# qiskit-community/adapt-aqc

Hardware: AMD Instinct MI355X
Metric: overlap+gradient evals/sec, 50-qubit MPS chi=64, 1/2/4/8 MI355X (higher is better)
Workload: dtype c128

## Files before the change

### adaptaqc_amd/csrc/svd_gram.h

```cpp
#pragma once

constexpr int kGramMaxK = 128;
constexpr int kGramNarrowK = 64;
constexpr double kGramRelFloor = 1e-9;
__device__ unsigned long long g_gram_ticks[12];
static_assert(kGramNarrowK == 64, "S5: the narrow inverse iteration (tid < K) stays on wave 0");
__device__ unsigned long long g_gram_stats[6];

__device__ __forceinline__ double wave_sum_d(double v) {
#pragma unroll
  for (int off = 32; off > 0; off >>= 1) v += __shfl_xor(v, off);
  return v;
}

__device__ __forceinline__ double wave_sum_dpp(double v) {
  v = aqc::row_sum16(v);
  double s = 0.0;
#pragma unroll
  for (int rr = 0; rr < 4; ++rr) {
    const int lo = __builtin_amdgcn_readlane(__double2loint(v), 16 * rr);
    const int hi = __builtin_amdgcn_readlane(__double2hiint(v), 16 * rr);
    s += __hiloint2double(hi, lo);
  }
  return s;
}

__device__ __forceinline__ cplx pick16(const cplx (&g)[16], int i) {
  switch (i) {
#define AQC_PICK(n) \
  case n:           \
    return g[n];
    AQC_PICK(0) AQC_PICK(1) AQC_PICK(2) AQC_PICK(3) AQC_PICK(4) AQC_PICK(5) AQC_PICK(6) AQC_PICK(7)
    AQC_PICK(8) AQC_PICK(9) AQC_PICK(10) AQC_PICK(11) AQC_PICK(12) AQC_PICK(13) AQC_PICK(14)
#undef AQC_PICK
    default:
      return g[15];
  }
}

__device__ __forceinline__ double uniform_d(double v) {
  const int lo = __builtin_amdgcn_readfirstlane(__double2loint(v));
  const int hi = __builtin_amdgcn_readfirstlane(__double2hiint(v));
  return __hiloint2double(hi, lo);
}

__device__ __forceinline__ double bcast_d(double v, int l) {
  const int lo = __builtin_amdgcn_readlane(__double2loint(v), l);
  const int hi = __builtin_amdgcn_readlane(__double2hiint(v), l);
  return __hiloint2double(hi, lo);
}

__device__ __forceinline__ int fresh_lane() {
  int l = __builtin_amdgcn_mbcnt_hi(~0u, __builtin_amdgcn_mbcnt_lo(~0u, 0u));
  asm volatile("" : "+v"(l));
  return l;
}
template <class T>
__device__ __forceinline__ T* uniform_ptr(T* p) {
  const unsigned long long a = (unsigned long long)p;
  const unsigned lo = __builtin_amdgcn_readfirstlane((unsigned)a);
  const unsigned hi = __builtin_amdgcn_readfirstlane((unsigned)(a >> 32));
  return (T*)(((unsigned long long)hi << 32) | lo);
}
__device__ __forceinline__ int sign_bit(double q) { return (int)((unsigned)__double2hiint(q) >> 31); }

__device__ __forceinline__ int sturm_count_poly(const double2* de, int C, double xn) {
  double p0 = 1.0, p1 = de[0].x - xn;
  int s1 = __double2hiint(p1) >> 31;
  int neg = s1;
  int i = 1;
  auto step = [&](double2 e) {
    const double p2 = fma(e.x - xn, p1, -(e.y * p0));
    const int s2 = __double2hiint(p2) >> 31;
    neg += s1 ^ s2;
    s1 = s2;
    p0 = p1;
    p1 = p2;
  };
  auto rescale = [&]() {
    const int ex = max(__builtin_amdgcn_frexp_exp(p0), __builtin_amdgcn_frexp_exp(p1));
    p0 = __builtin_amdgcn_ldexp(p0, -ex);
    p1 = __builtin_amdgcn_ldexp(p1, -ex);
  };
  auto rd4 = [&](int i0, double2& r0, double2& r1, double2& r2, double2& r3) {
    r0 = de[min(i0, C - 1)], r1 = de[min(i0 + 1, C - 1)], r2 = de[min(i0 + 2, C - 1)], r3 = de[min(i0 + 3, C - 1)];
  };
  double2 a0, a1, a2, a3, b0, b1, b2, b3;
  rd4(1, a0, a1, a2, a3);
  for (; i + 8 <= C; i += 8) {
    rd4(i + 4, b0, b1, b2, b3);
    __builtin_amdgcn_sched_barrier(0);
    step(a0);
    step(a1);
    step(a2);
    step(a3);
    rescale();
    rd4(i + 8, a0, a1, a2, a3);
    __builtin_amdgcn_sched_barrier(0);
    step(b0);
    step(b1);
    step(b2);
    step(b3);
    rescale();
  }
  if (i + 4 <= C) {
    step(a0);
    step(a1);
    step(a2);
    step(a3);
    rescale();
    i += 4;
  }
  for (; i < C; ++i) step(de[i]);
  return -neg;
}

__device__ __forceinline__ double rcp_nr(double x) {
  double r = __builtin_amdgcn_rcp(x);
  r = r * fma(-x, r, 2.0);
  r = r * fma(-x, r, 2.0);
  return r;
}

constexpr size_t kTfacOff = 16384;
constexpr size_t kWideOff = 20480;
static_assert(kWideOff + 8192 <= aqc::kGramWorkElems, "Gram-path scratch exceeds the work buffer");
static_assert(kChainLdsBytes >= 128 * 128 * 8, "S5 (K > 64): 128 x 128 vectors in the dynamic LDS");
typedef __attribute__((address_space(1))) double gdbl_t;

__device__ __forceinline__ void s6_factors(int b, int C, cplx* hh, const cplx* s_tau, int lane) {
  const int k1 = C - 1 - 16 * b, k0 = k1 > 16 ? k1 - 16 : 0, nb = k1 - k0;
  const int li = lane & 15, lk = lane >> 4;
  aqc::d4_t sr = {0, 0, 0, 0}, si = {0, 0, 0, 0};
  for (int r0 = 0; r0 < C; r0 += 4) {
    const int row = r0 + lk, k = k0 + li;
    const cplx y = (li < nb && row > k && row < C) ? aqc::ldg(hh + (size_t)k * (2 * C - k - 1) / 2 + (row - k - 1))
                                                   : aqc::cmk(0, 0);
    sr = __builtin_amdgcn_mfma_f64_16x16x4f64(y.x, y.x, sr, 0, 0, 0);
    sr = __builtin_amdgcn_mfma_f64_16x16x4f64(y.y, y.y, sr, 0, 0, 0);
    si = __builtin_amdgcn_mfma_f64_16x16x4f64(y.x, y.y, si, 0, 0, 0);
    si = __builtin_amdgcn_mfma_f64_16x16x4f64(-y.y, y.x, si, 0, 0, 0);
  }
  cplx* Sg = hh + kTfacOff + (size_t)b * 512;
#pragma unroll
  for (int q = 0; q < 4; ++q) aqc::stg(Sg + (lk + 4 * q) * 16 + li, aqc::cmk(sr[q], si[q]));
  asm volatile("s_waitcnt vmcnt(0)" ::: "memory");
  const int a = lane >> 2, g = lane & 3;
  cplx tq[4] = {aqc::cmk(0, 0), aqc::cmk(0, 0), aqc::cmk(0, 0), aqc::cmk(0, 0)};
  for (int i = 0; i < 16; ++i) {
    const cplx tau = i < nb ? s_tau[k0 + i] : aqc::cmk(0, 0);
    cplx acc = aqc::cmk(0, 0);
#pragma unroll
    for (int m = 0; m < 4; ++m) {
      const int bb = g + 4 * m;
      if (4 * m < i && bb < i) {
        const gdbl_t* sp = (const gdbl_t*)(const double*)(Sg + bb * 16 + i);
        const cplx sv = aqc::cmk(__hip_atomic_load(sp, __ATOMIC_RELAXED, __HIP_MEMORY_SCOPE_AGENT),
                                 __hip_atomic_load(sp + 1, __ATOMIC_RELAXED, __HIP_MEMORY_SCOPE_AGENT));
        acc = aqc::cfma(tq[m], sv, acc);
      }
    }
    acc.x = aqc::row_sum4(acc.x);
    acc.y = aqc::row_sum4(acc.y);
    const cplx ti = aqc::cmul(tau, acc);
    const cplx val = a < i ? aqc::cmk(-ti.x, -ti.y) : (a == i ? tau : aqc::cmk(0, 0));
    if (g == (i & 3)) tq[i >> 2] = val;
  }
#pragma unroll
  for (int m = 0; m < 4; ++m) aqc::stg(Sg + 256 + a * 16 + g + 4 * m, tq[m]);
}

template <int ZS>
__device__ __forceinline__ void gs_clusters(int K, int C, double* zb, const double* s_lam, double s_tn, int lane) {
  const double ortol = 1e-7 * s_tn;
  int start = 0;
  for (int i = 1; i < K; ++i) {
    if (s_lam[i - 1] - s_lam[i] >= ortol) {
      start = i;
      continue;
    }
    for (int jj = start; jj < i; ++jj) {
      double dp = 0.0;
      for (int row = lane; row < C; row += 64) dp = fma(zb[row * ZS + i], zb[row * ZS + jj], dp);
      dp = wave_sum_d(dp);
      for (int row = lane; row < C; row += 64) zb[row * ZS + i] = fma(-dp, zb[row * ZS + jj], zb[row * ZS + i]);
    }
    double n2 = 0.0;
    for (int row = lane; row < C; row += 64) n2 = fma(zb[row * ZS + i], zb[row * ZS + i], n2);
    n2 = wave_sum_d(n2);
    const double sc = 1.0 / sqrt(n2);
    for (int row = lane; row < C; row += 64) zb[row * ZS + i] *= sc;
  }
}

template <int ZS>
__device__ __forceinline__ double rayleigh(int i, int C, const double* zb, const double* s_d, const double* s_e) {
  double s2a = 0.0, s2b = 0.0;
  int r0 = 0;
  constexpr int U = 8;
  for (; r0 + U <= C; r0 += U) {
    double zz[U + 1], dd[U], ee[U];
#pragma unroll
    for (int u = 0; u <= U; ++u) zz[u] = zb[min(r0 + u, C - 1) * ZS + i];
#pragma unroll
    for (int u = 0; u < U; ++u) dd[u] = s_d[r0 + u], ee[u] = r0 + u < C - 1 ? s_e[r0 + u] : 0.0;
#pragma unroll
    for (int u = 0; u < U; ++u) {
      s2a = fma(dd[u] * zz[u], zz[u], s2a);
      s2b = fma(2.0 * ee[u] * zz[u], zz[u + 1], s2b);
    }
  }
  for (; r0 < C; ++r0) {
    const double z = zb[r0 * ZS + i];
    s2a = fma(s_d[r0] * z, z, s2a);
    if (r0 < C - 1) s2b = fma(2.0 * s_e[r0] * z, zb[(r0 + 1) * ZS + i], s2b);
  }
  const double s2 = s2a + s2b;
  return s2 > 0.0 ? s2 : 0.0;
}

__device__ __forceinline__ void s6_back(const TwoSiteJob& j, cplx* hh, int C, int K, int c0, aqc::d4_t (&vre)[2],
                                        aqc::d4_t (&vim)[2], const double* s_sig2, int tid, int lane, int wave,
                                        int wave_s) {
  extern __shared__ double2 xbuf[];
  const int nt = wave & 3, mg = wave >> 2, li = lane & 15, lk = lane >> 4;
  cplx* Yl = xbuf;
  cplx* Pw = Yl + 2048;
  cplx* Tl = Pw + 12 * 256;
  cplx* W2l = Tl + 3 * 256 + 16 * 64;
  auto fetch_y = [&](int k0, int nb, cplx (&y)[2]) {
#pragma unroll
    for (int u = 0; u < 2; ++u) {
      const int e = tid + 1024 * u, row = e >> 4, i = e & 15, k = k0 + i;
      y[u] = (i < nb && row > k && row < C) ? aqc::ldg(hh + (size_t)k * (2 * C - k - 1) / 2 + (row - k - 1))
                                            : aqc::cmk(0, 0);
    }
  };
  cplx ynx[2];
  {
    const int k1 = C - 1, k0 = k1 > 16 ? k1 - 16 : 0;
    fetch_y(k0, k1 - k0, ynx);
  }
  __syncthreads();
  for (int k1 = C - 1; k1 > 0; k1 -= 16) {
    const int k0 = k1 > 16 ? k1 - 16 : 0;
#pragma unroll
    for (int u = 0; u < 2; ++u) {
      const int e = tid + 1024 * u, row = e >> 4, i = e & 15;
      Yl[row * 16 + (i ^ (row & 15))] = ynx[u];
    }
    if (tid < 256) {
      const gdbl_t* tp = (const gdbl_t*)(const double*)(hh + kTfacOff + (size_t)((C - 1 - k1) >> 4) * 512 + 256 + tid);
      Tl[(tid >> 4) * 17 + (tid & 15)] = aqc::cmk(__hip_atomic_load(tp, __ATOMIC_RELAXED, __HIP_MEMORY_SCOPE_AGENT),
                                                  __hip_atomic_load(tp + 1, __ATOMIC_RELAXED, __HIP_MEMORY_SCOPE_AGENT));
    }
    __syncthreads();
    aqc::d4_t wr, wi;
    {
      aqc::d4_t p1 = {0, 0, 0, 0}, p2 = {0, 0, 0, 0}, p3 = {0, 0, 0, 0};
#pragma unroll
      for (int t = 0; t < 2; ++t) {
        if (32 * mg + 16 * t + 15 > k0) {
#pragma unroll
          for (int s = 0; s < 4; ++s) {
            const int row = 32 * mg + 16 * t + 4 * s + lk;
            const cplx y = Yl[row * 16 + (li ^ (row & 15))];
            p1 = __builtin_amdgcn_mfma_f64_16x16x4f64(y.x, vre[t][s], p1, 0, 0, 0);
            p2 = __builtin_amdgcn_mfma_f64_16x16x4f64(-y.y, vim[t][s], p2, 0, 0, 0);
            p3 = __builtin_amdgcn_mfma_f64_16x16x4f64(y.x - y.y, vre[t][s] + vim[t][s], p3, 0, 0, 0);
          }
        }
      }
#pragma unroll
      for (int q = 0; q < 4; ++q) wr[q] = p1[q] - p2[q], wi[q] = p3[q] - p1[q] - p2[q];
    }
    if (mg > 0) {
#pragma unroll
      for (int q = 0; q < 4; ++q) Pw[((mg - 1) * 4 + nt) * 256 + (lk + 4 * q) * 16 + li] = aqc::cmk(wr[q], wi[q]);
    }
    __syncthreads();
    if (mg == 0) {
      aqc::d4_t br, bi, p1 = {0, 0, 0, 0}, p2 = {0, 0, 0, 0}, p3 = {0, 0, 0, 0};
#pragma unroll
      for (int q = 0; q < 4; ++q) {
        const int b = lk + 4 * q;
        cplx w = aqc::cmk(wr[q], wi[q]);
#pragma unroll
        for (int m = 0; m < 3; ++m) w = aqc::cadd(w, Pw[(m * 4 + nt) * 256 + b * 16 + li]);
        br[q] = w.x;
        bi[q] = w.y;
      }
#pragma unroll
      for (int q = 0; q < 4; ++q) {
        const cplx t = Tl[li * 17 + 4 * q + lk];
        p1 = __builtin_amdgcn_mfma_f64_16x16x4f64(t.x, br[q], p1, 0, 0, 0);
        p2 = __builtin_amdgcn_mfma_f64_16x16x4f64(t.y, bi[q], p2, 0, 0, 0);
        p3 = __builtin_amdgcn_mfma_f64_16x16x4f64(t.x + t.y, br[q] + bi[q], p3, 0, 0, 0);
      }
#pragma unroll
      for (int q = 0; q < 4; ++q) W2l[(lk + 4 * q) * 64 + 16 * nt + li] = aqc::cmk(p1[q] - p2[q], p3[q] - p1[q] - p2[q]);
    }
    __syncthreads();
    if (k0 > 0) {
      const int n1 = k0, n0 = n1 > 16 ? n1 - 16 : 0;
      fetch_y(n0, n1 - n0, ynx);
    }
    const int vl_ = fresh_lane();
    const int vmg = wave_s >> 2, vnt = wave_s & 3, vli = vl_ & 15, vlk = vl_ >> 4;
#pragma unroll
    for (int t = 0; t < 2; ++t) {
      if (32 * vmg + 16 * t + 15 > k0) {
        const int row = 32 * vmg + 16 * t + vli;
        aqc::d4_t p1 = {0, 0, 0, 0}, p2 = {0, 0, 0, 0};
#pragma unroll
        for (int s = 0; s < 4; ++s) {
          const int b = 4 * s + vlk;
          const cplx y = Yl[row * 16 + (b ^ (row & 15))];
          const cplx w = W2l[b * 64 + 16 * vnt + vli];
          p1 = __builtin_amdgcn_mfma_f64_16x16x4f64(y.x, w.x, p1, 0, 0, 0);
          p2 = __builtin_amdgcn_mfma_f64_16x16x4f64(y.y, w.y, p2, 0, 0, 0);
          vim[t] = __builtin_amdgcn_mfma_f64_16x16x4f64(-(y.x + y.y), w.x + w.y, vim[t], 0, 0, 0);
        }
#pragma unroll
        for (int q = 0; q < 4; ++q) vre[t][q] += p2[q] - p1[q], vim[t][q] += p1[q] + p2[q];
      }
    }
    __syncthreads();
  }
  {
    const int col = c0 + 16 * nt + li;
    if (col < K) {
      const double sg = sqrt(s_sig2[col]);
#pragma unroll
      for (int t = 0; t < 2; ++t) {
#pragma unroll
        for (int q = 0; q < 4; ++q) {
          const int row = 32 * mg + 16 * t + lk + 4 * q;
          if (row < C) aqc::stg(j.work + (size_t)col * C + row, aqc::cmk(vre[t][q] * sg, vim[t][q] * sg));
        }
      }
    }
  }
}

__device__ __noinline__ void s5_wide(int i, int C, const double* s_d, const double* s_e, const double* s_e2,
                                     double lam, double tn, double* zb, double* Db) {
  for (int row = 0; row < C; ++row) {
    unsigned int h = (unsigned int)(row * 2654435761u) ^ (unsigned int)((i + 1) * 40503u);
    h ^= h >> 13;
    h *= 0x5bd1e995u;
    h ^= h >> 15;
    zb[row * 128 + i] = (double)(h & 0xFFFFFu) * (2.0 / 1048576.0) - 1.0;
  }
  auto ldd = [&](int row) {
    return __hip_atomic_load((const gdbl_t*)(Db + row * 128 + i), __ATOMIC_RELAXED, __HIP_MEMORY_SCOPE_AGENT);
  };
  constexpr int U = 8;
  const double itn = 1.0 / fmax(tn, 1e-300), lamn = lam * itn;
  {
    double p0 = 0.0, p1 = 1.0;
    for (int row = 0; row < C; ++row) {
      const double d = s_d[row], e2 = s_e2[max(row - 1, 0)];
      const double dmx = fma(d, itn, -lamn), t = (e2 * itn * itn) * p0;
      const double lim = 2.220446049250313e-16 * fabs(p1);
      double p = fma(dmx, p1, -t);
      p = fabs(p) < lim ? copysign(lim, p) : p;
      aqc::stg(Db + row * 128 + i, p1 * rcp_nr(p) * itn);
      p0 = p1;
      p1 = p;
      if ((row & 7) == 7) {
        const int ex = max(__builtin_amdgcn_frexp_exp(p0), __builtin_amdgcn_frexp_exp(p1));
        p0 = __builtin_amdgcn_ldexp(p0, -ex);
        p1 = __builtin_amdgcn_ldexp(p1, -ex);
      }
    }
  }
  asm volatile("s_waitcnt vmcnt(0)" ::: "memory");
  double sc = 1.0;
  for (int it = 0; it < 3; ++it) {
    double yp = 0.0;
    int r0 = 0;
    for (; r0 + U <= C; r0 += U) {
      double zz[U], ee[U], dp[U];
#pragma unroll
      for (int u = 0; u < U; ++u) {
        const int rm = max(r0 + u - 1, 0);
        zz[u] = zb[(r0 + u) * 128 + i], ee[u] = s_e[rm], dp[u] = ldd(rm);
      }
#pragma unroll
      for (int u = 0; u < U; ++u) {
        const double y = fma(-ee[u] * dp[u], yp, zz[u] * sc);
        zb[(r0 + u) * 128 + i] = y;
        yp = y;
      }
    }
    for (; r0 < C; ++r0) {
      const int rm = max(r0 - 1, 0);
      const double y = fma(-s_e[rm] * ldd(rm), yp, zb[r0 * 128 + i] * sc);
      zb[r0 * 128 + i] = y;
      yp = y;
    }
    double zn = 0.0, n2 = 0.0;
    int r1 = C - 1;
    for (; r1 - U + 1 >= 0; r1 -= U) {
      double yy[U], ee[U], dd[U];
#pragma unroll
      for (int u = 0; u < U; ++u) {
        const int row = r1 - u;
        yy[u] = zb[row * 128 + i], ee[u] = s_e[min(row, C - 2)], dd[u] = ldd(row);
      }
#pragma unroll
      for (int u = 0; u < U; ++u) {
        zn = fma(-ee[u] * dd[u], zn, yy[u] * dd[u]);
        zb[(r1 - u) * 128 + i] = zn;
        n2 = fma(zn, zn, n2);
      }
    }
    for (; r1 >= 0; --r1) {
      const double d = ldd(r1);
      zn = fma(-s_e[min(r1, C - 2)] * d, zn, zb[r1 * 128 + i] * d);
      zb[r1 * 128 + i] = zn;
      n2 = fma(zn, zn, n2);
    }
    const double rs = __builtin_amdgcn_rsq(n2);
    sc = rs * fma(-0.5 * n2 * rs, rs, 1.5);
  }
  for (int row = 0; row < C; ++row) zb[row * 128 + i] *= sc;
}

__device__ __noinline__ void gram_wide(const TwoSiteJob& j, cplx* hh, int C, int K, const double* s_d,
                                       const double* s_e, const double* s_e2, const double* s_lam, double s_tn,
                                       const cplx* s_tau, double* s_sig2) {
  extern __shared__ double2 xbuf[];
  const int tid = fresh_tid(), lane = tid & 63, wave = tid >> 6;
  const int wave_s = __builtin_amdgcn_readfirstlane(wave);
  double* zb = reinterpret_cast<double*>(xbuf);
  double* scratch = reinterpret_cast<double*>(j.work + kWideOff);
  const int nblk = (C - 1 + 15) >> 4;
  if (tid < K) {
    s5_wide(tid, C, s_d, s_e, s_e2, s_lam[tid], s_tn, zb, scratch);
  } else if ((wave & 3) >= 2) {
    const int b = 2 * (wave >> 2) + (wave & 3) - 2;
    if (b < nblk) s6_factors(b, C, hh, s_tau, lane);
  }
  __syncthreads();
  if (wave == 0) gs_clusters<128>(K, C, zb, s_lam, s_tn, lane);
  __syncthreads();
  if (tid < K) s_sig2[tid] = rayleigh<128>(tid, C, zb, s_d, s_e);
  __syncthreads();
  const int nt = wave & 3, mg = wave >> 2, li = lane & 15, lk = lane >> 4;
  for (int pass = 0; pass < 2; ++pass) {
    const int c0 = pass == 0 ? kGramNarrowK : 0;
    aqc::d4_t vre[2], vim[2];
#pragma unroll
    for (int t = 0; t < 2; ++t) {
#pragma unroll
      for (int q = 0; q < 4; ++q) {
        const int row = 32 * mg + 16 * t + lk + 4 * q, col = 16 * nt + li;
        double v = 0.0;
        if (row < C && c0 + col < K)
          v = pass == 0 ? zb[row * 128 + c0 + col]
                        : __hip_atomic_load((const gdbl_t*)(scratch + row * 64 + col), __ATOMIC_RELAXED,
                                            __HIP_MEMORY_SCOPE_AGENT);
        vre[t][q] = v;
        vim[t][q] = 0.0;
      }
    }
    if (pass == 0)
      for (int e = tid; e < C * 64; e += 1024) aqc::stg(scratch + e, zb[(e >> 6) * 128 + (e & 63)]);
    s6_back(j, hh, C, K, c0, vre, vim, s_sig2, tid, lane, wave, wave_s);
  }
}

__device__ __noinline__ double gram_cert128(const TwoSiteJob& j, int C, int K, const double* sig2) {
  extern __shared__ double2 xbuf[];
  __shared__ double red[16];
  const int tid = fresh_tid(), sg = tid >> 8, lt = tid & 255, wave = lt >> 6, lane = tid & 63;
  const int M = 2 * j.dims[0], N = 2 * j.dims[2];
  const bool tr = M < N;
  const int L = tr ? N : M;
  const cplx* th = j.theta;
  const cplx* W = j.work;
  cplx* Y = j.work + 16384;
  static_assert(16384 + 128 * 128 <= aqc::kGramWorkElems, "certificate scratch");
  auto xel = [&](int R, int c) { return tr ? aqc::cconj(aqc::ldg(th + (size_t)R * M + c)) : aqc::ldg(th + (size_t)c * M + R); };
  auto lda = [](const cplx* p) {
    const gdbl_t* q = (const gdbl_t*)(const double*)p;
    return aqc::cmk(__hip_atomic_load(q, __ATOMIC_RELAXED, __HIP_MEMORY_SCOPE_AGENT),
                    __hip_atomic_load(q + 1, __ATOMIC_RELAXED, __HIP_MEMORY_SCOPE_AGENT));
  };
  aqc::GemmLds& lds = reinterpret_cast<aqc::GemmLds*>(xbuf)[sg];
  const int bi = 64 * (sg >> 1), bj = 64 * (sg & 1);
  const int wr = (wave >> 1) * 32, wc = (wave & 1) * 32, li = lane & 15, lk = lane >> 4;
  aqc::d4_t cr[2][2], ci[2][2];
  aqc::block_cgemm_tile<false, false, false>(
      L, K, C, bi, bj, [&](int R, int c) { return xel(R, c); },
      [&](int c, int k) { return aqc::cscale(lda(W + (size_t)k * C + c), 1.0 / sqrt(sig2[k])); }, lds, lt,
      bi < L && bj < K, cr, ci);
#pragma unroll
  for (int r = 0; r < 2; ++r)
#pragma unroll
    for (int c = 0; c < 2; ++c)
#pragma unroll
      for (int q = 0; q < 4; ++q) {
        const int row = bi + wr + 16 * r + lk + 4 * q, col = bj + wc + 16 * c + li;
        if (row < L && col < K) aqc::stg(Y + (size_t)row * 128 + col, aqc::cmk(cr[r][c][q], ci[r][c][q]));
      }
  __syncthreads();
  aqc::block_cgemm_tile<false, false, false>(
      L, C, K, bi, bj, [&](int R, int k) { return lda(Y + (size_t)R * 128 + k); },
      [&](int k, int c) { return aqc::cscale(aqc::cconj(lda(W + (size_t)k * C + c)), 1.0 / sqrt(sig2[k])); }, lds,
      lt, bi < L && bj < C, cr, ci);
  double acc = 0.0;
#pragma unroll
  for (int r = 0; r < 2; ++r)
#pragma unroll
    for (int c = 0; c < 2; ++c)
#pragma unroll
      for (int q = 0; q < 4; ++q) {
        const int row = bi + wr + 16 * r + lk + 4 * q, col = bj + wc + 16 * c + li;
        if (row < L && col < C) {
          const cplx x = xel(row, col);
          const double dx = x.x - cr[r][c][q], dy = x.y - ci[r][c][q];
          acc = fma(dx, dx, fma(dy, dy, acc));
        }
      }
  acc = wave_sum_dpp(acc);
  if (lane == 0) red[tid >> 6] = acc;
  __syncthreads();
  double t = 0.0;
#pragma unroll
  for (int w = 0; w < 16; ++w) t += red[w];
  __syncthreads();
  return t;
}

#ifndef AQC_S3_TAIL
#define AQC_S3_TAIL 0
#endif
constexpr int kS3Tail = 32;
#if defined(__HIP_DEVICE_COMPILE__)
using s3_lcplx = __attribute__((address_space(3))) cplx;
using s3_ldbl = __attribute__((address_space(3))) double;
#else
using s3_lcplx = cplx;
using s3_ldbl = double;
#endif
__device__ __forceinline__ void s3_tail(cplx (&g)[16], int C, int r0, int q0, int tid, int lane, int wave,
                                        s3_lcplx* lb, cplx* hh) {
  const int T0 = C - kS3Tail;
  s3_lcplx* pvb = lb;
  s3_lcplx* vbb = lb + 256;
  s3_lcplx* tauS = lb + 1921;
  s3_ldbl* eS = (s3_ldbl*)(lb + 2050);
  s3_ldbl* dS = (s3_ldbl*)(lb + 2114);
  s3_lcplx* a2b = lb + 2178;
  s3_lcplx* tile = lb + 2304;
  s3_lcplx* vt = lb + 2304 + 32 * 33;
  s3_lcplx* pt = vt + 32;
  {
    const int bp = (T0 - 1) & 1;
    const int r = r0, q = q0;
    if (r >= T0 && r < C) {
      const cplx vr = vbb[bp * 128 + r], pr = pvb[bp * 128 + r];
      const double a2r2 = 2.0 * a2b[bp].x;
      const cplx wr = aqc::cmk(fma(a2r2, vr.x, pr.x), fma(a2r2, vr.y, pr.y));
#pragma unroll
      for (int i = 0; i < 16; ++i) {
        const int c = q + 8 * i;
        if (c >= T0 && c < C) {
          const cplx vc = vbb[bp * 128 + c], pc = pvb[bp * 128 + c];
          cplx x = g[i];
          x.x = fma(-vr.x, pc.x, fma(-vr.y, pc.y, fma(-wr.x, vc.x, fma(-wr.y, vc.y, x.x))));
          x.y = fma(-vr.y, pc.x, fma(vr.x, pc.y, fma(-wr.y, vc.x, fma(wr.x, vc.y, x.y))));
          tile[(r - T0) * 33 + (c - T0)] = x;
        }
      }
    }
  }
  __syncthreads();
  if (wave == 0) {
    const int rr = lane >> 1, h = lane & 1;
#pragma unroll
    for (int i = 0; i < 16; ++i) g[i] = tile[rr * 33 + 2 * i + h];
    for (int kk = 0; kk < kS3Tail - 1; ++kk) {
      const int K = T0 + kk;
      cplx x = h == (kk & 1) ? pick16(g, kk >> 1) : aqc::cmk(0, 0);
      x.x += __shfl_xor(x.x, 1);
      x.y += __shfl_xor(x.y, 1);
      const double xn2 = wave_sum_dpp(h == 0 && rr > kk + 1 ? aqc::cnorm2(x) : 0.0);
      const double dkk = bcast_d(x.x, 2 * kk);
      const cplx alpha = aqc::cmk(bcast_d(x.x, 2 * (kk + 1)), bcast_d(x.y, 2 * (kk + 1)));
      const double x2 = fma(alpha.x, alpha.x, fma(alpha.y, alpha.y, xn2));
      double rs = __builtin_amdgcn_rsq(x2);
      rs = rs * fma(-0.5 * x2 * rs, rs, 1.5);
      rs = rs * fma(-0.5 * x2 * rs, rs, 1.5);
      const double nn = x2 * rs;
      const bool triv = xn2 == 0.0 && alpha.y == 0.0;
      const double beta = triv ? alpha.x : (alpha.x >= 0.0 ? -nn : nn);
      const double ib = alpha.x >= 0.0 ? -rs : rs;
      const double dr = alpha.x - beta, di = alpha.y, id2 = rcp_nr(fma(dr, dr, di * di));
      const cplx tau = triv ? aqc::cmk(0, 0) : aqc::cmk((beta - alpha.x) * ib, -alpha.y * ib);
      const cplx scl = triv ? aqc::cmk(0, 0) : aqc::cmk(dr * id2, -di * id2);
      cplx v = rr > kk + 1 ? aqc::cmul(x, scl) : aqc::cmk(rr == kk + 1 ? 1.0 : 0.0, 0.0);
      if (lane == 0) {
        tauS[K] = tau;
        eS[K] = beta;
        dS[K] = dkk;
      }
      if (h == 0) {
        vt[rr] = v;
        if (rr > kk) aqc::stg(hh + (size_t)K * (2 * C - K - 1) / 2 + (T0 + rr - K - 1), v);
      }
      __builtin_amdgcn_fence(__ATOMIC_RELEASE, "workgroup");
      cplx acc = aqc::cmk(0, 0);
#pragma unroll
      for (int i = 0; i < 16; ++i)
        if (2 * i + 1 > kk) acc = aqc::cfma(g[i], vt[2 * i + h], acc);
      acc.x += __shfl_xor(acc.x, 1);
      acc.y += __shfl_xor(acc.y, 1);
      const cplx p = rr > kk ? aqc::cmul(tau, acc) : aqc::cmk(0, 0);
      const double ktx = wave_sum_dpp(h == 0 ? fma(p.x, v.x, p.y * v.y) : 0.0);
      const double kty = wave_sum_dpp(h == 0 ? fma(p.x, v.y, -p.y * v.x) : 0.0);
      const cplx a2 = aqc::cscale(aqc::cmul(tau, aqc::cmk(ktx, kty)), -0.5);
      if (h == 0) pt[rr] = p;
      __builtin_amdgcn_fence(__ATOMIC_RELEASE, "workgroup");
      const double a2r2 = 2.0 * a2.x;
      const cplx w = aqc::cmk(fma(a2r2, v.x, p.x), fma(a2r2, v.y, p.y));
#pragma unroll
      for (int i = 0; i < 16; ++i) {
        if (2 * i + 1 > kk) {
          const cplx pc = pt[2 * i + h], vci = vt[2 * i + h];
          g[i].x = fma(-v.x, pc.x, fma(-v.y, pc.y, fma(-w.x, vci.x, fma(-w.y, vci.y, g[i].x))));
          g[i].y = fma(-v.y, pc.x, fma(v.x, pc.y, fma(-w.y, vci.x, fma(w.x, vci.y, g[i].y))));
        }
      }
    }
    const cplx glast = pick16(g, (kS3Tail - 1) >> 1);
    const double dl = bcast_d(glast.x, 2 * (kS3Tail - 1) + ((kS3Tail - 1) & 1));
    if (lane == 0) dS[C - 1] = dl;
  }
}

#ifndef AQC_GRAM_INLINE
#define AQC_GRAM_INLINE 0
#endif
#if AQC_GRAM_INLINE
__device__ __forceinline__
#else
__device__ __noinline__
#endif
int gram_svd_body(const TwoSiteJob& j) {
  extern __shared__ double2 xbuf[];
  __shared__ double s_d[128], s_e[128], s_e2[128], s_lam[128], s_err[128], s_sig2[kGramMaxK], s_tail;
  __shared__ int s_K, s_cert;
  __shared__ cplx s_tau[128];
  __shared__ double s_lo, s_hi, s_tn;
  __shared__ double2 s_de[128];
  const int chl = j.dims[0], chr = j.dims[2];
  const int M = 2 * chl, N = 2 * chr;
  const bool tr = M < N;
  const int L = tr ? N : M, C = tr ? M : N;
  const int KE = (j.max_chi > 0 && j.max_chi < C) ? j.max_chi : C;
  const int tid = fresh_tid(), lane = tid & 63, wave = tid >> 6;
  const int wave_s = __builtin_amdgcn_readfirstlane(wave);
  if (tid == 0) atomicAdd(&g_gram_stats[0], 1ull);
  if (C < 4 || C > 128 || L > 128 || j.cap < 64) {
    if (tid == 0) atomicAdd(&g_gram_stats[2], 1ull);
    return 0;
  }
  const cplx* th = j.theta;
  unsigned long long t_last = tid == 0 ? __builtin_amdgcn_s_memtime() : 0ull;
  auto tick = [&](int ph) {
    if (tid == 0) {
      const unsigned long long t = __builtin_amdgcn_s_memtime();
      atomicAdd(&g_gram_ticks[ph], t - t_last);
      t_last = t;
    }
  };
  unsigned long long t_a = 0, t_b = 0;
  auto tick_step = [&](unsigned long long& acc) {
    if (tid == 0) {
      const unsigned long long t = __builtin_amdgcn_s_memtime();
      acc += t - t_last;
      t_last = t;
    }
  };
  const int r0 = tid >> 3, q0 = tid & 7;
  const int r = r0, q = q0;
  cplx g[16];
  {
    constexpr int KC = 8, PITCH = 144;
    constexpr int ARR = KC * PITCH, BUF = 4 * ARR;
    double* sb = reinterpret_cast<double*>(xbuf);
    const int nt = (C + 15) >> 4, ntile = nt * (nt + 1) / 2;
    int tI[3], tJ[3];
    bool tact[3];
    const bool rs = nt == 8;
    if (rs) {
      constexpr unsigned kTab[16] = {0x300, 0x322, 0x333, 0x355, 0x330, 0x352, 0x241, 0x244,
                                     0x311, 0x260, 0x261, 0x264, 0x000, 0x177, 0x263, 0x266};
      const unsigned e = kTab[wave];
#pragma unroll
      for (int u = 0; u < 3; ++u) {
        tact[u] = u < (int)(e >> 8);
        tI[u] = e & 15;
        tJ[u] = ((e >> 4) & 15) + u;
      }
    } else {
#pragma unroll
      for (int u = 0; u < 3; ++u) {
        int t = wave + 16 * u, ti = 0;
        tact[u] = t < ntile;
        while (tact[u] && t >= nt - ti) t -= nt - ti++;
        tI[u] = ti;
        tJ[u] = ti + t;
      }
    }
    const int nch = (L + KC - 1) / KC;
    auto fetch = [&](int ch) {
      const int kk = ch * KC + (tr ? tid >> 7 : tid & 7), c = tr ? tid & 127 : tid >> 3;
      if (kk >= L || c >= C) return aqc::cmk(0, 0);
      return tr ? aqc::ldg(th + (size_t)kk * M + c) : aqc::ldg(th + (size_t)c * M + kk);
    };
    auto stash = [&](int buf, cplx x) {
      if (tr) x.y = -x.y;
      const int o = buf * BUF + (tr ? tid >> 7 : tid & 7) * PITCH + (tr ? tid & 127 : tid >> 3);
      sb[o] = x.x;
      sb[o + ARR] = x.y;
      sb[o + 2 * ARR] = x.x + x.y;
      sb[o + 3 * ARR] = x.x - x.y;
    };
    aqc::d4_t p1[3], p2[3], p3[3];
#pragma unroll
    for (int u = 0; u < 3; ++u) p1[u] = p2[u] = p3[u] = aqc::d4_t{0, 0, 0, 0};
    stash(0, fetch(0));
    __syncthreads();
    for (int ch = 0; ch < nch; ++ch) {
      const bool more = ch + 1 < nch;
      cplx xn = aqc::cmk(0, 0);
      if (more) xn = fetch(ch + 1);
      const double* cb = sb + (ch & 1) * BUF;
      const int fl = fresh_lane();
#pragma unroll
      for (int ks = 0; ks < KC / 4; ++ks) {
        const int row = (4 * ks + (fl >> 4)) * PITCH + (fl & 15);
        if (rs) {
          const int oi = row + 16 * tI[0];
          const double ar = cb[oi], ai = cb[ARR + oi], as = cb[2 * ARR + oi];
#pragma unroll
          for (int u = 0; u < 3; ++u) {
            if (tact[u]) {
              const int oj = row + 16 * tJ[u];
              p1[u] = __builtin_amdgcn_mfma_f64_16x16x4f64(ar, cb[oj], p1[u], 0, 0, 0);
              p2[u] = __builtin_amdgcn_mfma_f64_16x16x4f64(ai, cb[ARR + oj], p2[u], 0, 0, 0);
              p3[u] = __builtin_amdgcn_mfma_f64_16x16x4f64(as, cb[3 * ARR + oj], p3[u], 0, 0, 0);
            }
          }
        } else {
#pragma unroll
          for (int u = 0; u < 3; ++u) {
            if (tact[u]) {
              const int oi = row + 16 * tI[u], oj = row + 16 * tJ[u];
              p1[u] = __builtin_amdgcn_mfma_f64_16x16x4f64(cb[oi], cb[oj], p1[u], 0, 0, 0);
              p2[u] = __builtin_amdgcn_mfma_f64_16x16x4f64(cb[ARR + oi], cb[ARR + oj], p2[u], 0, 0, 0);
              p3[u] = __builtin_amdgcn_mfma_f64_16x16x4f64(cb[2 * ARR + oi], cb[3 * ARR + oj], p3[u], 0, 0, 0);
            }
          }
        }
      }
      if (more) stash((ch + 1) & 1, xn);
      __syncthreads();
    }
    cplx* gsq = xbuf;
    auto up_index = [](int a, int b) {
      if (b < 64) return 64 * 65 + b * (b + 1) / 2 + a;
      if (a >= 64) return 64 * 65 + 2080 + (b - 64) * (b - 63) / 2 + (a - 64);
      return a * 65 + (b - 64);
    };
#pragma unroll
    for (int u = 0; u < 3; ++u) {
      if (tact[u]) {
#pragma unroll
        for (int qq = 0; qq < 4; ++qq) {
          const int a = 16 * tI[u] + (lane >> 4) + 4 * qq, b = 16 * tJ[u] + (lane & 15);
          if (a <= b && b < C)
            gsq[up_index(a, b)] = aqc::cmk(p1[u][qq] + p2[u][qq], p1[u][qq] - p2[u][qq] - p3[u][qq]);
        }
      }
    }
    __syncthreads();
#pragma unroll
    for (int i = 0; i < 16; ++i) {
      const int c = q + 8 * i, rw = r;
      cplx v = aqc::cmk(0, 0);
      if (rw < C && c < C) {
        v = gsq[c >= rw ? up_index(rw, c) : up_index(c, rw)];
        if (c < rw) v.y = -v.y;
      }
      g[i] = v;
    }
    __syncthreads();
  }
  tick(0);
  cplx* hh = uniform_ptr(j.work);
#if defined(__HIP_DEVICE_COMPILE__)
  using lcplx = __attribute__((address_space(3))) cplx;
  using ldbl = __attribute__((address_space(3))) double;
#else
  using lcplx = cplx;
  using ldbl = double;
#endif
  lcplx* lb = (lcplx*)xbuf;
  asm volatile("" : "+s"(lb));
  lcplx* pvb = lb;
  lcplx* vbb = lb + 256;
  lcplx* xvb = lb + 512;
  lcplx* accp = lb + 768;
  lcplx* gk1b = lb + 1792;
  lcplx* tauS = lb + 1921;
  ldbl* eS = (ldbl*)(lb + 2050);
  ldbl* dS = (ldbl*)(lb + 2114);
  lcplx* a2b = lb + 2178;
  lcplx* scal = lb + 2180;
  lcplx* ktp = lb + 2183;
  volatile __attribute__((address_space(3))) int* hsf =
      (volatile __attribute__((address_space(3))) int*)(lb + 2185);
  if (tid == 0) {
    tauS[-1] = aqc::cmk(0, 0);
    a2b[1] = aqc::cmk(0, 0);
    hsf[0] = hsf[1] = 0;
  }
  if (q == 0) {
    pvb[128 + r] = aqc::cmk(0, 0);
    vbb[128 + r] = aqc::cmk(0, 0);
    xvb[128 + r] = (r > 0 && r < C) ? g[0] : aqc::cmk(0, 0);
  }
  __syncthreads();
  const bool s3tail = AQC_S3_TAIL && C >= 64;
  const int kEnd = s3tail ? C - kS3Tail : C - 1;
  for (int k = 0; k < kEnd; ++k) {
    const int b = k & 1, bp = b ^ 1;
    int q = q0, r = r0;
    asm volatile("" : "+v"(q), "+v"(r));
    const bool wact = wave * 8 + 7 >= k;
    double a2x = 0.0;
    if (wact) a2x = uniform_d(a2b[bp].x);
    if (wave == 0) {
      __builtin_amdgcn_s_setprio(3);
      double xn2;
      {
        const cplx x0 = xvb[bp * 128 + lane], x1 = xvb[bp * 128 + 64 + lane];
        const double n0 = lane > k + 1 ? aqc::cnorm2(x0) : 0.0, n1 = lane + 64 > k + 1 ? aqc::cnorm2(x1) : 0.0;
        xn2 = wave_sum_dpp(n0 + n1);
      }
      const cplx alpha = xvb[bp * 128 + k + 1];
      const double x2 = fma(alpha.x, alpha.x, fma(alpha.y, alpha.y, xn2));
      double rs = __builtin_amdgcn_rsq(x2);
      rs = rs * fma(-0.5 * x2 * rs, rs, 1.5);
      rs = rs * fma(-0.5 * x2 * rs, rs, 1.5);
      const double nn = x2 * rs;
      const bool triv = xn2 == 0.0 && alpha.y == 0.0;
      const double beta = triv ? alpha.x : (alpha.x >= 0.0 ? -nn : nn);
      const double ib = alpha.x >= 0.0 ? -rs : rs;
      const double dr = alpha.x - beta, di = alpha.y, id2 = rcp_nr(fma(dr, dr, di * di));
      const cplx tau = triv ? aqc::cmk(0, 0) : aqc::cmk((beta - alpha.x) * ib, -alpha.y * ib);
      const cplx scl = triv ? aqc::cmk(0, 0) : aqc::cmk(dr * id2, -di * id2);
      if (lane == 0) {
        tauS[k] = tau;
        eS[k] = beta;
        scal[0] = scl;
        scal[1] = aqc::cmul(tau, scl);
      }
      __builtin_amdgcn_s_setprio(0);
    }
    if (wact) {
      cplx acc = aqc::cmk(0, 0);
      const cplx vr = vbb[bp * 128 + r];
      const cplx pr = pvb[bp * 128 + r];
      const double a2r2 = 2.0 * a2x;
      const cplx wr = aqc::cmk(fma(a2r2, vr.x, pr.x), fma(a2r2, vr.y, pr.y));
      const double nvx = -vr.x, nvy = -vr.y, nwx = -wr.x, nwy = -wr.y;
      auto col = [&](int i, const cplx& vc, const cplx& pc, const cplx& xc) {
        g[i].x = fma(nvx, pc.x, fma(nvy, pc.y, fma(nwx, vc.x, fma(nwy, vc.y, g[i].x))));
        g[i].y = fma(nvy, pc.x, fma(vr.x, pc.y, fma(nwy, vc.x, fma(wr.x, vc.y, g[i].y))));
        acc = aqc::cfma(g[i], xc, acc);
      };
#ifndef AQC_S3_GROUP
#define AQC_S3_GROUP 2
#endif
      constexpr int GR = AQC_S3_GROUP;
      const int gi0 = k / (8 * GR);
      cplx cv, cp, cz;
      {
        const int c = q + 8 * GR * gi0;
        cv = vbb[bp * 128 + c], cp = pvb[bp * 128 + c], cz = xvb[bp * 128 + c];
      }
#pragma unroll
      for (int gi = 0; gi < 16 / GR; ++gi) {
        if (gi >= gi0) {
#pragma unroll
          for (int ii = 0; ii < GR; ++ii) {
            const int i = GR * gi + ii;
            cplx nv = cv, np = cp, nz = cz;
            if (i + 1 < 16) {
              const int c = q + 8 * (i + 1);
              nv = vbb[bp * 128 + c], np = pvb[bp * 128 + c], nz = xvb[bp * 128 + c];
            }
            __builtin_amdgcn_sched_barrier(0);
            col(i, cv, cp, cz);
            cv = nv, cp = np, cz = nz;
          }
        }
      }
      cplx gk = pick16(g, k >> 3);
      asm volatile("" : "+v"(gk.x), "+v"(gk.y));
      const cplx gk1 = ((k + 1) & 7) ? gk : pick16(g, (k + 1) >> 3);
      if (q == (k & 7) && r == k) dS[k] = gk.x;
      acc.x = aqc::row_sum8(acc.x);
      acc.y = aqc::row_sum8(acc.y);
      if (q == 0) accp[r] = acc;
      if (q == ((k + 1) & 7)) gk1b[r] = gk1;
    }
    __syncthreads();
    tick_step(t_b);
    if (wave < 2) {
      int rr = tid;
      asm volatile("" : "+v"(rr));
      const double beta = eS[k];
      const cplx ts = scal[1], scl = scal[0];
      const cplx g1 = gk1b[rr];
      cplx sum = accp[rr];
      sum.x = fma(-beta, g1.x, sum.x);
      sum.y = fma(-beta, g1.y, sum.y);
      const bool rowact = rr > k && rr < C, below = rr > k + 1 && rr < C;
      cplx p = aqc::cmul(ts, sum);
      if (!rowact) p = aqc::cmk(0, 0);
      cplx v = aqc::cmul(xvb[bp * 128 + rr], scl);
      if (!below) v = aqc::cmk(rr == k + 1 ? 1.0 : 0.0, 0.0);
      pvb[b * 128 + rr] = p;
      vbb[b * 128 + rr] = v;
      if (rowact) aqc::stg(hh + (size_t)k * (2 * C - k - 1) / 2 + (rr - k - 1), v);
      xvb[b * 128 + rr] = below ? aqc::csub(g1, p) : aqc::cmk(0, 0);
      const double ktx = wave_sum_dpp(fma(p.x, v.x, p.y * v.y)), kty = wave_sum_dpp(fma(p.x, v.y, -p.y * v.x));
      if (lane == 0) ktp[wave] = aqc::cmk(ktx, kty);
      __builtin_amdgcn_fence(__ATOMIC_RELEASE, "workgroup");
      if (lane == 0) hsf[wave] = k + 1;
      while (hsf[wave ^ 1] != k + 1) __builtin_amdgcn_s_sleep(1);
      __builtin_amdgcn_fence(__ATOMIC_ACQUIRE, "workgroup");
      const cplx a2 = aqc::cscale(aqc::cmul(tauS[k], aqc::cadd(ktp[0], ktp[1])), -0.5);
      const cplx pk = pvb[b * 128 + k + 1];
      const double sx = -(pk.x + 2.0 * a2.x), sy = pk.y;
      int r2 = tid;
      asm volatile("" : "+v"(r2));
      if (r2 > k + 1 && r2 < C) xvb[b * 128 + r2] = aqc::cfma(aqc::cmk(sx, sy), vbb[b * 128 + r2], xvb[b * 128 + r2]);
      if (tid == 0) a2b[b] = a2;
    }
    __syncthreads();
    tick_step(t_a);
  }
  if (s3tail) {
    s3_tail(g, C, r0, q0, tid, lane, wave, lb, hh);
  } else
  if (wave == (C - 1) >> 3) {
    const int bp = (C - 2) & 1;
    const cplx a2 = a2b[bp];
    const bool own = r0 == C - 1 && q0 == ((C - 1) & 7);
    const int gi = (C - 1) >> 3;
    if (own) {
      const cplx v = vbb[bp * 128 + C - 1], p = pvb[bp * 128 + C - 1];
      const cplx w = aqc::cfma(a2, v, p);
      const cplx gl = pick16(g, gi);
      dS[C - 1] = gl.x - 2.0 * (v.x * w.x + v.y * w.y);
    }
  }
  __syncthreads();
  for (int i = tid; i < C; i += 1024) {
    s_d[i] = dS[i];
    if (i < C - 1) {
      s_e[i] = eS[i];
      s_tau[i] = tauS[i];
    }
  }
  __syncthreads();
  if (tid == 0) {
    atomicAdd(&g_gram_ticks[6], t_a + t_b);
    atomicAdd(&g_gram_ticks[8], t_b);
  }
  tick(1);
  if (wave == 0) {
    double lo = 1e300, hi = -1e300, tn = 0.0;
    for (int i = lane; i < C; i += 64) {
      const double el = i > 0 ? fabs(s_e[i - 1]) : 0.0, er = i < C - 1 ? fabs(s_e[i]) : 0.0;
      const double di = s_d[i];
      lo = fmin(lo, di - el - er);
      hi = fmax(hi, di + el + er);
      tn = fmax(tn, fabs(di) + el + er);
      if (i < C - 1) s_e2[i] = s_e[i] * s_e[i];
      s_de[i] = make_double2(di, i > 0 ? s_e[i - 1] * s_e[i - 1] : 0.0);
    }
#pragma unroll
    for (int off = 32; off > 0; off >>= 1) {
      lo = fmin(lo, __shfl_xor(lo, off));
      hi = fmax(hi, __shfl_xor(hi, off));
      tn = fmax(tn, __shfl_xor(tn, off));
    }
    if (lane == 0) {
      const double span = fmax(hi - lo, 1e-300);
      s_lo = lo - 1e-12 * span;
      s_hi = hi + 1e-12 * span;
      s_tn = tn;
    }
    const double itn = 1.0 / fmax(tn, 1e-300);
    for (int i = lane; i < C; i += 64) {
      const double2 de = s_de[i];
      s_de[i] = make_double2(de.x * itn, de.y * itn * itn);
    }
  }
  __syncthreads();
  {
    constexpr int kG = 4, kFirst = 256, kRounds = 12;
    static_assert(kG == 4 || kG == 8 || kG == 16, "lanes per eigenvalue");
    const int eid = tid / kG, sub = tid % kG;
    const int a = C - 1 - eid;
    int* cntb = reinterpret_cast<int*>(xbuf);
    const double lo0 = s_lo, span0 = s_hi - s_lo;
    const double itn = 1.0 / fmax(s_tn, 1e-300);
    constexpr double kInvF = 1.0 / (kFirst + 1), kInvG = 1.0 / (kG + 1);
    if (tid < kFirst) cntb[tid] = sturm_count_poly(s_de, C, (lo0 + span0 * (double)(tid + 1) * kInvF) * itn);
    __syncthreads();
    const int rounds = kRounds + (j.thr > 1e-12 * s_tn ? 3 : 0);
    if (tid < KE * kG) {
      double lo, hi;
      {
        int l = 0, h = kFirst;
        while (l < h) {
          const int m = (l + h) >> 1;
          if (cntb[m] >= a + 1) h = m;
          else l = m + 1;
        }
        lo = l > 0 ? lo0 + span0 * (double)l * kInvF : s_lo;
        hi = l < kFirst ? lo0 + span0 * (double)(l + 1) * kInvF : s_hi;
      }
      for (int round = 0; round < rounds; ++round) {
        const double x = lo + (hi - lo) * (double)(sub + 1) * kInvG;
        const int cnt = sturm_count_poly(s_de, C, x * itn);
        const unsigned long long bal = __ballot(cnt >= a + 1);
        const unsigned int gm = (unsigned int)(bal >> (lane & ~(kG - 1))) & ((1u << kG) - 1u);
        const int f = gm ? __builtin_ctz(gm) : kG;
        const double nhi = f < kG ? lo + (hi - lo) * (double)(f + 1) * kInvG : hi;
        const double nlo = f > 0 ? lo + (hi - lo) * (double)f * kInvG : lo;
        lo = nlo;
        hi = nhi;
      }
      if (sub == 0) {
        s_lam[eid] = 0.5 * (lo + hi);
        s_err[eid] = 0.5 * (hi - lo);
      }
    }
  }
  __syncthreads();
  if (tid == 0) s_K = aqc::gram_keep(s_lam, s_err, KE, C, j.max_chi, j.thr, s_tn, kGramRelFloor, s_tail, &s_cert);
  __syncthreads();
  tick(2);
  const int K = s_K;
  if (K < 0) {
    if (tid == 0) atomicAdd(&g_gram_stats[3], 1ull);
    return 0;
  }
  if (K > kGramNarrowK) {
    gram_wide(j, hh, C, K, s_d, s_e, s_e2, s_lam, s_tn, s_tau, s_sig2);
    tick(4);
  } else {
  double* zb = reinterpret_cast<double*>(xbuf);
  double* Db = zb + 128 * 64;
  if (tid < K) {
    const int i = tid;
    const double lam = s_lam[i];
    const double piv = 2.220446049250313e-16 * s_tn;
    for (int row = 0; row < C; ++row) {
      unsigned int h = (unsigned int)(row * 2654435761u) ^ (unsigned int)((i + 1) * 40503u);
      h ^= h >> 13;
      h *= 0x5bd1e995u;
      h ^= h >> 15;
      zb[row * 64 + i] = (double)(h & 0xFFFFFu) * (2.0 / 1048576.0) - 1.0;
    }
    constexpr int U = 8;
    (void)piv;
    const double itn = 1.0 / fmax(s_tn, 1e-300), lamn = lam * itn;
    double p0 = 0.0, p1 = 1.0;
    auto fac_row = [&](int row, double d, double e2, double& unused) {
      (void)unused;
      const double dmx = fma(d, itn, -lamn), t = (e2 * itn * itn) * p0;
      const double lim = 2.220446049250313e-16 * fabs(p1);
      double p = fma(dmx, p1, -t);
      p = fabs(p) < lim ? copysign(lim, p) : p;
      Db[row * 64 + i] = p1 * rcp_nr(p) * itn;
      p0 = p1;
      p1 = p;
    };
    {
      double rdp = 0.0;
      int r0 = 0;
      for (; r0 + U <= C; r0 += U) {
        double dd[U], ee[U];
#pragma unroll
        for (int u = 0; u < U; ++u) dd[u] = s_d[r0 + u], ee[u] = s_e2[max(r0 + u - 1, 0)];
#pragma unroll
        for (int u = 0; u < U; ++u) fac_row(r0 + u, dd[u], ee[u], rdp);
        const int ex = max(__builtin_amdgcn_frexp_exp(p0), __builtin_amdgcn_frexp_exp(p1));
        p0 = __builtin_amdgcn_ldexp(p0, -ex);
        p1 = __builtin_amdgcn_ldexp(p1, -ex);
      }
      for (; r0 < C; ++r0) fac_row(r0, s_d[r0], s_e2[max(r0 - 1, 0)], rdp);
    }
    double sc = 1.0;
    for (int it = 0; it < 3; ++it) {
      double yp = 0.0;
      auto fwd_row = [&](int row, double z, double e, double dp) {
        const double y = fma(-e * dp, yp, z * sc);
        zb[row * 64 + i] = y;
        yp = y;
      };
      int r0 = 0;
      for (; r0 + U <= C; r0 += U) {
        double zz[U], ee[U], dp[U];
#pragma unroll
        for (int u = 0; u < U; ++u) {
          const int rm = max(r0 + u - 1, 0);
          zz[u] = zb[(r0 + u) * 64 + i], ee[u] = s_e[rm], dp[u] = Db[rm * 64 + i];
        }
#pragma unroll
        for (int u = 0; u < U; ++u) fwd_row(r0 + u, zz[u], ee[u], dp[u]);
      }
      for (; r0 < C; ++r0) {
        const int rm = max(r0 - 1, 0);
        fwd_row(r0, zb[r0 * 64 + i], s_e[rm], Db[rm * 64 + i]);
      }
      double zn = 0.0, n2 = 0.0;
      auto bwd_row = [&](int row, double y, double e, double d) {
        zn = fma(-e * d, zn, y * d);
        zb[row * 64 + i] = zn;
        n2 = fma(zn, zn, n2);
      };
      int r1 = C - 1;
      for (; r1 - U + 1 >= 0; r1 -= U) {
        double yy[U], ee[U], dd[U];
#pragma unroll
        for (int u = 0; u < U; ++u) {
          const int row = r1 - u;
          yy[u] = zb[row * 64 + i], ee[u] = s_e[min(row, C - 2)], dd[u] = Db[row * 64 + i];
        }
#pragma unroll
        for (int u = 0; u < U; ++u) bwd_row(r1 - u, yy[u], ee[u], dd[u]);
      }
      for (; r1 >= 0; --r1) bwd_row(r1, zb[r1 * 64 + i], s_e[min(r1, C - 2)], Db[r1 * 64 + i]);
      const double rs = __builtin_amdgcn_rsq(n2);
      sc = rs * fma(-0.5 * n2 * rs, rs, 1.5);
    }
    {
      int r0 = 0;
      for (; r0 + U <= C; r0 += U) {
        double zz[U];
#pragma unroll
        for (int u = 0; u < U; ++u) zz[u] = zb[(r0 + u) * 64 + i];
#pragma unroll
        for (int u = 0; u < U; ++u) zb[(r0 + u) * 64 + i] = zz[u] * sc;
      }
      for (; r0 < C; ++r0) zb[r0 * 64 + i] *= sc;
    }
    if (tid == 0) atomicAdd(&g_gram_ticks[7], __builtin_amdgcn_s_memtime() - t_last);
  }
  else if ((wave & 3) != 0 && wave - 1 - (wave >> 2) < ((C - 1 + 15) >> 4)) {
    s6_factors(wave - 1 - (wave >> 2), C, hh, s_tau, lane);
  }
  __syncthreads();
  if (wave == 0) gs_clusters<64>(K, C, zb, s_lam, s_tn, lane);
  __syncthreads();
  if (tid < K) s_sig2[tid] = rayleigh<64>(tid, C, zb, s_d, s_e);
  __syncthreads();
  tick(3);
  const int nt = wave & 3, mg = wave >> 2, li = lane & 15, lk = lane >> 4;
  aqc::d4_t vre[2], vim[2];
#pragma unroll
  for (int t = 0; t < 2; ++t) {
#pragma unroll
    for (int q = 0; q < 4; ++q) {
      const int row = 32 * mg + 16 * t + lk + 4 * q, col = 16 * nt + li;
      vre[t][q] = (row < C && col < K) ? zb[row * 64 + col] : 0.0;
      vim[t][q] = 0.0;
    }
  }
  s6_back(j, hh, C, K, 0, vre, vim, s_sig2, tid, lane, wave, wave_s);
  tick(4);
  }
  for (int c = tid; c < C; c += 1024) aqc::stg(j.sig + c, c < K ? sqrt(s_sig2[c]) : 0.0);
  if (tid == 0) aqc::stg(j.sig + kSigTail, s_tail);
  tick(5);
  if (s_cert) return 2;
  if (tid == 0) {
    atomicMax(&j.flags[2], 1);
    atomicAdd(&g_gram_stats[1], 1ull);
  }
  return 1;
}

__device__ __noinline__ bool gram_certified(const TwoSiteJob& j) {
  const int tid = fresh_tid();
  __shared__ double s_s2[128];
  __shared__ int s_k;
  const int M = 2 * j.dims[0], N = 2 * j.dims[2], C = M < N ? M : N;
  if (tid == 0) s_k = 0;
  __syncthreads();
  if (tid < C) {
    const double sg = aqc::ldg(j.sig + tid);
    s_s2[tid] = sg * sg;
    if (sg > 0.0) atomicMax(&s_k, tid + 1);
  }
  __syncthreads();
  if (tid == 0) atomicAdd(&g_gram_stats[4], 1ull);
  const double cs = gram_cert128(j, C, s_k, s_s2);
  const bool ok = cs < 0.5 * aqc::kReduceChop;
  if (tid == 0) {
    atomicAdd(&g_gram_stats[ok ? 5 : 3], 1ull);
    if (ok) {
      atomicMax(&j.flags[2], 1);
      atomicAdd(&g_gram_stats[1], 1ull);
    } else {
      aqc::stg(j.sig + kSigTail, 0.0);
    }
  }
  __syncthreads();
  return ok;
}

__global__ __launch_bounds__(1024) void k_svd_gram(const TwoSiteJob* __restrict__ jobs) {
  const TwoSiteJob& j = jobs[blockIdx.x];
  const int g = j.gram ? gram_svd_body(j) : 0;
  if (g == 1) return;
  __syncthreads();
  if (g == 2 && gram_certified(j)) return;
  jacobi_reg_body<128, 8, 16>(j);
}
```

Before: 8.118 million.

## Replace inter-wave LDS handshake with redundant per-wave computation of partner rows

In the Householder tridiagonalization step, each of the two active waves now loads and computes its partner wave's 64 rows (rr^64) as well as its own. It then forms the full dot product locally and broadcasts the pivot value itself. This removes the LDS flag spin-wait, the fences and the ktp exchange between waves, and fuses the final xvb update into a single store. The cost is roughly double the arithmetic and LDS reads per wave. It also depends on a wave_s symbol and a bcast_d helper that must already exist.

```diff
diff --git a/adaptaqc_amd/csrc/svd_gram.h b/adaptaqc_amd/csrc/svd_gram.h
--- a/adaptaqc_amd/csrc/svd_gram.h
+++ b/adaptaqc_amd/csrc/svd_gram.h
@@ -823,13 +823,9 @@
   ldbl* dS = (ldbl*)(lb + 2114);
   lcplx* a2b = lb + 2178;
   lcplx* scal = lb + 2180;
-  lcplx* ktp = lb + 2183;
-  volatile __attribute__((address_space(3))) int* hsf =
-      (volatile __attribute__((address_space(3))) int*)(lb + 2185);
   if (tid == 0) {
     tauS[-1] = aqc::cmk(0, 0);
     a2b[1] = aqc::cmk(0, 0);
-    hsf[0] = hsf[1] = 0;
   }
   if (q == 0) {
     pvb[128 + r] = aqc::cmk(0, 0);
@@ -927,33 +923,40 @@
     if (wave < 2) {
       int rr = tid;
       asm volatile("" : "+v"(rr));
+      const int ro = rr ^ 64;
       const double beta = eS[k];
-      const cplx ts = scal[1], scl = scal[0];
-      const cplx g1 = gk1b[rr];
-      cplx sum = accp[rr];
-      sum.x = fma(-beta, g1.x, sum.x);
-      sum.y = fma(-beta, g1.y, sum.y);
+      const cplx ts = scal[1], scl = scal[0], tau = tauS[k];
+      const cplx g1 = gk1b[rr], g1o = gk1b[ro];
+      cplx sum = accp[rr], so = accp[ro];
+      const cplx xo = xvb[bp * 128 + rr], xt = xvb[bp * 128 + ro];
+      __builtin_amdgcn_sched_barrier(0);
+      sum.x = fma(-beta, g1.x, sum.x), sum.y = fma(-beta, g1.y, sum.y);
+      so.x = fma(-beta, g1o.x, so.x), so.y = fma(-beta, g1o.y, so.y);
+      const bool kown = wave_s == ((k + 1) >> 6);
+      const int kl = (k + 1) & 63;
+      const cplx sk = aqc::cmk(bcast_d(kown ? sum.x : so.x, kl), bcast_d(kown ? sum.y : so.y, kl));
+      const cplx pk = aqc::cmul(ts, sk);
       const bool rowact = rr > k && rr < C, below = rr > k + 1 && rr < C;
       cplx p = aqc::cmul(ts, sum);
       if (!rowact) p = aqc::cmk(0, 0);
-      cplx v = aqc::cmul(xvb[bp * 128 + rr], scl);
+      cplx v = aqc::cmul(xo, scl);
       if (!below) v = aqc::cmk(rr == k + 1 ? 1.0 : 0.0, 0.0);
+      double ktx, kty;
+      {
+        cplx po = aqc::cmul(ts, so);
+        if (!(ro > k && ro < C)) po = aqc::cmk(0, 0);
+        cplx vo = aqc::cmul(xt, scl);
+        if (!(ro > k + 1 && ro < C)) vo = aqc::cmk(ro == k + 1 ? 1.0 : 0.0, 0.0);
+        const double ox = wave_sum_dpp(fma(po.x, vo.x, po.y * vo.y)), oy = wave_sum_dpp(fma(po.x, vo.y, -po.y * vo.x));
+        ktx = wave_sum_dpp(fma(p.x, v.x, p.y * v.y)) + ox;
+        kty = wave_sum_dpp(fma(p.x, v.y, -p.y * v.x)) + oy;
+      }
+      const cplx a2 = aqc::cscale(aqc::cmul(tau, aqc::cmk(ktx, kty)), -0.5);
+      const double sx = -(pk.x + 2.0 * a2.x), sy = pk.y;
       pvb[b * 128 + rr] = p;
       vbb[b * 128 + rr] = v;
       if (rowact) aqc::stg(hh + (size_t)k * (2 * C - k - 1) / 2 + (rr - k - 1), v);
-      xvb[b * 128 + rr] = below ? aqc::csub(g1, p) : aqc::cmk(0, 0);
-      const double ktx = wave_sum_dpp(fma(p.x, v.x, p.y * v.y)), kty = wave_sum_dpp(fma(p.x, v.y, -p.y * v.x));
-      if (lane == 0) ktp[wave] = aqc::cmk(ktx, kty);
-      __builtin_amdgcn_fence(__ATOMIC_RELEASE, "workgroup");
-      if (lane == 0) hsf[wave] = k + 1;
-      while (hsf[wave ^ 1] != k + 1) __builtin_amdgcn_s_sleep(1);
-      __builtin_amdgcn_fence(__ATOMIC_ACQUIRE, "workgroup");
-      const cplx a2 = aqc::cscale(aqc::cmul(tauS[k], aqc::cadd(ktp[0], ktp[1])), -0.5);
-      const cplx pk = pvb[b * 128 + k + 1];
-      const double sx = -(pk.x + 2.0 * a2.x), sy = pk.y;
-      int r2 = tid;
-      asm volatile("" : "+v"(r2));
-      if (r2 > k + 1 && r2 < C) xvb[b * 128 + r2] = aqc::cfma(aqc::cmk(sx, sy), vbb[b * 128 + r2], xvb[b * 128 + r2]);
+      xvb[b * 128 + rr] = below ? aqc::cfma(aqc::cmk(sx, sy), v, aqc::csub(g1, p)) : aqc::cmk(0, 0);
       if (tid == 0) a2b[b] = a2;
     }
     __syncthreads();
```

Result: no change. 8.154 million (median of 6 runs) (+0.5%).
